# cmaestre/pcl_tracking

Measured on AMD Instinct MI355X. Metric: particles x input-points / sec per frame (tracked frames/sec @8192 particles per GPU), higher is better.
Workload: dtype f32

## Files before the change

include/pft.h:

```cpp
#ifndef PFT_H
#define PFT_H

#include <stddef.h>
#include <stdint.h>

#ifdef __cplusplus
extern "C" {
#endif

#define PFT_ABI_VERSION 5

typedef struct pft_point_xyzrgba {
  float x, y, z, w;
  uint32_t rgba;
  uint32_t pad[3];
} pft_point_xyzrgba;

typedef struct pft_particle {
  float x, y, z, w;
  float roll, pitch, yaw, weight;
} pft_particle;

typedef enum pft_status {
  PFT_OK = 0,
// ... 93 lines not shown
int pft_dist_begin_frame(pft_tracker* t);
int pft_dist_phase_a(pft_tracker* t, int iteration);
int pft_dist_phase_b(pft_tracker* t);
int pft_dist_phase_c(pft_tracker* t);

int pft_set_particles(pft_tracker* t, const pft_particle* p, size_t n);
int pft_eval_weights(pft_tracker* t, const pft_particle* particles, size_t P, float* raw_w, int32_t* nn_idx,
                     float* nn_d2);
int pft_debug_get_bbox(pft_tracker* t, float bbox[6]);
int pft_debug_get_crop(pft_tracker* t, int32_t* idx, size_t cap, size_t* n);
int pft_debug_get_octree(pft_tracker* t, int32_t* depth, double min_xyz[3], double max_xyz[3], uint32_t* n_leaves,
                         uint32_t* n_nodes);
int pft_debug_get_point_keys(pft_tracker* t, uint32_t* keys3, size_t cap_points);
int pft_debug_get_scan_stats(pft_tracker* t, uint64_t* queries, uint64_t* scanned_points);
int pft_debug_set_limits(pft_tracker* t, uint32_t max_words, int sorted_npass);
int pft_debug_state_save(pft_tracker* t);
int pft_debug_state_restore(pft_tracker* t);
int pft_debug_inject_error(pft_tracker* t, uint32_t bits);
int pft_debug_get_host_stat(pft_tracker* t, uint32_t out4[4]);
int pft_debug_get_ticks(pft_tracker* t, uint64_t* ticks32);
int pft_debug_get_descent_stats(pft_tracker* t, uint64_t* dbg32);
int pft_debug_get_hard_steps(pft_tracker* t, uint64_t out5[5]);
int pft_debug_get_likelihood_layout(pft_tracker* t, uint32_t out4[4]);
int pft_debug_aabb_support_subset(const pft_point_xyzrgba* pts, size_t n, uint32_t* keep, size_t* n_keep);
#ifdef PFT_DIAG
void pft_debug_set_ablate(pft_tracker* t, int mask);
#endif
int pft_debug_likelihood_occupancy(void);
int pft_debug_normalize(pft_tracker* t, float* w_inout, size_t n, double* fit_ratio);
int pft_debug_alias(pft_tracker* t, const float* w, size_t n, int32_t* a, double* q);
int pft_debug_weighted_mean(pft_tracker* t, const pft_particle* p, size_t n, pft_particle* out);
int pft_debug_init_particles(pft_tracker* t, const pft_particle* rep, uint32_t id_offset, size_t n_local,
                             pft_particle* out);
int pft_debug_resample(pft_tracker* t, const pft_particle* old, size_t n_total, const int32_t* a, const double* q,
                       const pft_particle* rep, uint32_t epoch, uint32_t id_offset, size_t n_local,
                       pft_particle* out);
int pft_debug_pose_to_matrix(pft_tracker* t, const pft_particle* p, size_t n, float* m12);
int pft_debug_kld_resample(pft_tracker* t, const pft_particle* old, size_t n_old, const int32_t* a, const double* q,
                           const pft_particle* motion, uint32_t epoch, pft_particle* out, int32_t* bins6,
                           uint32_t* n_out, uint32_t* k_out);
double pft_kld_normal_quantile(double u);
double pft_kld_bound(int k, double delta, double epsilon);

enum {
  PFT_K_RESAMPLE = 0, PFT_K_AABB = 1, PFT_K_CROP = 2, PFT_K_OCTREE = 3, PFT_K_LIKELIHOOD = 4,
  PFT_K_POPULATION = 5, PFT_K_PACK = 6, PFT_K_COUNT = 7
// ... 11 lines not shown
```

pcl_tracking_amd/_lib.py:

```python
import ctypes as C
import os

_HERE = os.path.dirname(os.path.abspath(__file__))
LIB_PATH = os.environ.get("PFT_LIB_PATH") or os.path.join(_HERE, "_build", "libpft_hip.so")

PFT_ABI_VERSION = 5
PFT_SUM_TREE, PFT_SUM_PCL = 0, 1
PFT_CD_RING = 32
K_RESAMPLE, K_AABB, K_CROP, K_OCTREE, K_LIKELIHOOD, K_POPULATION, K_PACK, K_COUNT = range(8)

STATUS = {0: "ok", 1: "invalid argument", 2: "no input cloud", 3: "no reference cloud", 4: "no usable HIP device",
          5: "HIP error", 6: "capacity exceeded", 7: "invalid state"}


class PftError(RuntimeError):
    def __init__(self, status, detail=""):
        self.status = status
        super().__init__("pft status %d (%s) %s" % (status, STATUS.get(status, "?"), detail))


class Config(C.Structure):
    _fields_ = [
        ("abi_version", C.c_uint32), ("device_id", C.c_int32), ("stream", C.c_void_p),
        ("stream_is_external", C.c_int32),
# ... 79 lines not shown
    ("pft_to_state", None, [_vp, _vp]),
    ("pft_get_fit_ratio", C.c_int, [_vp, _P(_f64)]),
    ("pft_synchronize", C.c_int, [_vp]),
    ("pft_dist_bind", C.c_int, [_vp, _vp, _vp, _vp]),
    ("pft_dist_begin_frame", C.c_int, [_vp]),
    ("pft_dist_phase_a", C.c_int, [_vp, C.c_int]),
    ("pft_dist_phase_b", C.c_int, [_vp]),
    ("pft_dist_phase_c", C.c_int, [_vp]),
    ("pft_set_particles", C.c_int, [_vp, _vp, _sz]),
    ("pft_eval_weights", C.c_int, [_vp, _vp, _sz, _vp, _vp, _vp]),
    ("pft_debug_get_bbox", C.c_int, [_vp, _vp]),
    ("pft_debug_get_crop", C.c_int, [_vp, _vp, _sz, _P(_sz)]),
    ("pft_debug_get_octree", C.c_int, [_vp, _P(_i32), _vp, _vp, _P(_u32), _P(_u32)]),
    ("pft_debug_get_point_keys", C.c_int, [_vp, _vp, _sz]),
    ("pft_debug_get_scan_stats", C.c_int, [_vp, _P(_u64), _P(_u64)]),
    ("pft_debug_set_limits", C.c_int, [_vp, _u32, C.c_int]),
    ("pft_debug_inject_error", C.c_int, [_vp, _u32]),
    ("pft_debug_state_save", C.c_int, [_vp]),
    ("pft_debug_state_restore", C.c_int, [_vp]),
    ("pft_debug_get_host_stat", C.c_int, [_vp, _vp]),
    ("pft_debug_get_ticks", C.c_int, [_vp, _vp]),
    ("pft_debug_get_descent_stats", C.c_int, [_vp, _vp]),
    ("pft_debug_get_likelihood_layout", C.c_int, [_vp, _vp]),
    ("pft_debug_get_hard_steps", C.c_int, [_vp, _vp]),
    ("pft_debug_aabb_support_subset", C.c_int, [_vp, C.c_size_t, _vp, _vp]),
    ("pft_debug_likelihood_occupancy", C.c_int, []),
    ("pft_debug_normalize", C.c_int, [_vp, _vp, _sz, _P(_f64)]),
    ("pft_debug_alias", C.c_int, [_vp, _vp, _sz, _vp, _vp]),
    ("pft_debug_weighted_mean", C.c_int, [_vp, _vp, _sz, _vp]),
    ("pft_debug_init_particles", C.c_int, [_vp, _vp, _u32, _sz, _vp]),
    ("pft_debug_resample", C.c_int, [_vp, _vp, _sz, _vp, _vp, _vp, _u32, _u32, _sz, _vp]),
    ("pft_debug_pose_to_matrix", C.c_int, [_vp, _vp, _sz, _vp]),
    ("pft_debug_kld_resample", C.c_int, [_vp, _vp, _sz, _vp, _vp, _vp, _u32, _vp, _vp, _P(_u32), _P(_u32)]),
    ("pft_set_change_detector", C.c_int, [_vp, C.c_int, C.c_int, C.c_int, _f64]),
    ("pft_get_change_detector", C.c_int, [_vp, _P(C.c_int), _P(C.c_int), _P(C.c_int), _P(_f64)]),
    ("pft_debug_change_state", C.c_int, [_vp, C.c_int, _P(_u32), _P(_u32), _vp, _P(_i32), _vp, _P(_u32)]),
    ("pft_debug_change_detect", C.c_int, [_vp, _vp, _sz, C.c_int, _f64, C.c_int, _vp, _sz, _P(_sz)]),
    ("pft_set_report_cloud", C.c_int, [_vp, _vp, _sz]),
    ("pft_report", C.c_int, [_vp]),
    ("pft_get_report", C.c_int, [_vp, _P(ObjectReport)]),
    ("pft_get_tracked_cloud", C.c_int, [_vp, _vp, _sz, _P(_sz)]),
    ("pft_kld_normal_quantile", _f64, [_f64]),
    ("pft_kld_bound", _f64, [C.c_int, _f64, _f64]),
    ("pft_profile_enable", C.c_int, [_vp, C.c_int]),
    ("pft_profile_get", C.c_int, [_vp, C.c_int, _P(_f64), _P(_u64)]),
    ("pft_profile_reset", C.c_int, [_vp]),
# ... 77 lines not shown
```

pcl_tracking_amd/csrc/pft_api.hip:

```cpp
#include <math.h>
#include <stdio.h>
#include <string.h>

#include <stdlib.h>

#include <algorithm>
#include <cmath>
#include <string>
#include <vector>

#include "pft_internal.h"

#define HIPCHK(t, call)                                                                       \
  do {                                                                                        \
    hipError_t e_ = (call);                                                                   \
    if (e_ != hipSuccess) {                                                                   \
      (t)->err = std::string(#call) + ": " + hipGetErrorString(e_);                           \
      return PFT_ERR_HIP;                                                                     \
    }                                                                                         \
  } while (0)

struct EvPair {
  hipEvent_t a, b;
};
// ... 13 lines not shown
  std::string err;

  pft_point_xyzrgba* d_ref_raw = nullptr;
  float4 *d_ref_xyz = nullptr, *d_ref_hsv = nullptr, *d_ref_box = nullptr;
  size_t bbox_part_cap = 0;
  uint32_t ref_cap = 0;
  pft_point_xyzrgba* d_in_raw = nullptr;
  float4* d_in_pts = nullptr;
  uint32_t in_cap = 0, N = 0;
  const pft_point_xyzrgba* raw_pending = nullptr;
  pft_particle* d_part[2] = {nullptr, nullptr};
  int cur = 0;
  float* d_mats = nullptr;
  float* d_bbox_part = nullptr;
  float* d_bbox6 = nullptr;
  uint32_t* d_crop_counts = nullptr;
  unsigned long long* d_crop_slots = nullptr;
  uint32_t crop_epoch = 0;
  float4* d_crop_pts = nullptr;
  int32_t* d_crop_idx = nullptr;
  uint32_t* d_words = nullptr;
  uint32_t max_words = 0;
  uint16_t* d_jump = nullptr;
  uint32_t* d_ref_perm = nullptr;
  float4* d_leaf_pts = nullptr;
  uint32_t *d_leaf_order = nullptr, *d_pt_node = nullptr, *d_pt_key = nullptr, *d_pt_tmp = nullptr;
  unsigned long long* d_pt_key64 = nullptr;
  SortBufs sort = {};
  uint32_t* h_stat = nullptr;
  PftSwitches sw = {};
  bool leaf_indirect = false;
  int force_npass = 0;
  uint32_t inject_error = 0;
  double* d_partial = nullptr;
  int32_t* d_alias_list = nullptr;
  double* d_alias_pref = nullptr;
  double* d_pop_part = nullptr;
  uint32_t *d_eg_start = nullptr, *d_eg_cnt = nullptr, *d_eg_tile = nullptr;
  uint32_t *d_ec_slot = nullptr, *d_ec_cells = nullptr, *d_ec_count = nullptr, *d_ec_base = nullptr;
  float4* d_ec_list = nullptr;
  uint32_t ec_pool_cap = 0;
  uint32_t *d_eq_cellq = nullptr, *d_eq_nq = nullptr, *d_eq_qbase = nullptr, *d_eq_bbase = nullptr, *d_eq_fill = nullptr,
           *d_eq_blk = nullptr, *d_eq_tiles = nullptr;
  float4* d_eq_sorted = nullptr;
  double* d_eq_out = nullptr;
  uint32_t eq_cap = 0, eq_blk_cap = 0, eq_tiles_cap = 0;
// ... 241 lines not shown
}

static void sync_dev(pft_tracker* t) {
  PftDev& d = t->dev;
  d.ref_xyz = t->d_ref_xyz;
  d.ref_box = t->d_ref_box;
  d.ref_hsv = t->d_ref_hsv;
  d.in_pts = t->d_in_pts;
  d.N = t->N;
  d.part_cur = t->d_part[t->cur];
  d.part_all = t->bound_gathered ? static_cast<pft_particle*>(t->bound_gathered) : t->d_part[t->cur];
  d.mats = t->d_mats;
  d.bbox_part = t->d_bbox_part;
  d.bbox_grid = (uint32_t)t->num_cus;
  d.bbox_part_cap = (uint32_t)t->bbox_part_cap;
  d.bbox6 = t->bound_bbox6 ? static_cast<float*>(t->bound_bbox6) : t->d_bbox6;
  d.crop_counts = t->d_crop_counts;
  d.crop_slots = t->d_crop_slots;
  d.crop_pts = t->d_crop_pts;
  d.crop_idx = t->d_crop_idx;
  d.words = t->d_words;
  d.max_words = t->max_words;
  d.jump = t->d_jump;
  d.ref_perm = t->d_ref_perm;
  d.leaf_pts = t->d_leaf_pts;
  d.leaf_order = t->d_leaf_order;
  d.pt_node = t->d_pt_node;
  d.pt_key = t->d_pt_key;
  d.pt_tmp = t->d_pt_tmp;
  d.pt_key64 = t->d_pt_key64;
  d.host_stat = t->h_stat;
  d.partial = t->d_partial;
  d.alias_list = t->d_alias_list;
  d.alias_pref = t->d_alias_pref;
  d.pop_part = t->d_pop_part;
  d.p_active = t->prm.kld ? &t->d_hdr->p_active : nullptr;
  d.eg_start = t->d_eg_start;
  d.eg_cnt = t->d_eg_cnt;
  d.eg_tile = t->d_eg_tile;
  d.eg_cap = t->d_eg_start ? PFT_EG_CAP : 0u;
  d.ec_slot = t->d_ec_slot;
  d.ec_cells = t->d_ec_cells;
  d.ec_count = t->d_ec_count;
  d.ec_base = t->d_ec_base;
  d.ec_list = t->d_ec_list;
  d.ec_pool_cap = t->ec_pool_cap;
// ... 119 lines not shown
      HIPCHK(t, hipMemcpyAsync(n.b.set_cnt[k], c.b.set_cnt[k], (size_t)c.b.cap * 4u, hipMemcpyDeviceToDevice, t->stream));
    }
    HIPCHK(t, hipStreamSynchronize(t->stream));
  } else {
    HIPCHK(t, hipMemsetAsync(n.b.st, 0, sizeof(PftChangeState), t->stream));
  }
  cd_free(c);
  c = n;
  return PFT_OK;
}

PftSwitches pft_read_switches() {
  auto on = [](const char* name) { return getenv(name) != nullptr; };
  auto is1 = [](const char* name) { const char* e = getenv(name); return e && e[0] == '1'; };
  PftSwitches w = {};
  w.graph = is1("PFT_GRAPH");
  if (const char* b = getenv("PFT_FORCE_BUILDER")) w.builder = !strcmp(b, "single") ? 1 : (!strcmp(b, "sorted") ? 2 : 0);
  w.leaf_indirect = on("PFT_LEAF_INDIRECT") ? (int)is1("PFT_LEAF_INDIRECT") : -1;
  w.aabb_full = on("PFT_AABB_FULL");
  w.resample_one_lane = on("PFT_RESAMPLE_ONE_LANE");
  w.split_resample = on("PFT_SPLIT_RESAMPLE") || w.resample_one_lane;
  w.crop_two_pass = on("PFT_CROP_TWO_PASS");
  w.generic_descent = is1("PFT_GENERIC_DESCENT");
  w.exact_path = on("PFT_EXACT_SHELLS_ONLY") ? PftExactPath::shells : on("PFT_EXACT_PER_QUERY") ? PftExactPath::per_query : PftExactPath::sorted;
#ifdef PFT_DIAG
  if (const char* a = getenv("PFT_ABLATE")) w.ablate = atoi(a);
  w.skip_octree = on("PFT_DEBUG_SKIP_OCTREE");
#endif
  return w;
}

#ifdef PFT_DIAG
extern "C" void pft_debug_set_ablate(pft_tracker* t, int mask) { if (t) t->sw.ablate = mask; }
#endif

extern "C" int pft_create(const pft_config* cfg, pft_tracker** out) {
  if (!cfg || !out) return PFT_ERR_INVALID_ARG;
  *out = nullptr;
  if (cfg->abi_version != PFT_ABI_VERSION || cfg->particle_num <= 0 || cfg->iteration_num <= 0 ||
      cfg->world_size <= 0 || cfg->rank < 0 || cfg->rank >= cfg->world_size || cfg->use_normal != 0 ||
      cfg->particle_num % cfg->world_size != 0 || !(cfg->octree_resolution > 0) ||
      (cfg->sum_order != PFT_SUM_TREE && cfg->sum_order != PFT_SUM_PCL))
    return PFT_ERR_INVALID_ARG;
  if (cfg->particle_num > PFT_MAX_PARTICLES) return PFT_ERR_CAPACITY;
  if (cfg->kld_adaptive) {
    if (cfg->world_size != 1 || cfg->maximum_particle_num <= 0 || !(cfg->kld_epsilon > 0)) return PFT_ERR_INVALID_ARG;
// ... 47 lines not shown
  p.M = 0;
  p.nchunk = 1;
  p.ref_chunk = PFT_REF_CHUNK;
  p.split_last = 0;
  p.kld = cfg->kld_adaptive ? 1u : 0u;
  p.kld_max = (uint32_t)cfg->maximum_particle_num;
  p.kld_z = pft_kld_normal_quantile(cfg->kld_delta);
  p.kld_eps = cfg->kld_epsilon;
  for (int k = 0; k < 6; k++) p.kld_bin[k] = (float)cfg->kld_bin_size[k];
  p.motion_ratio = cfg->motion_ratio;
  p.sum_order = cfg->sum_order;
  t->Pcap = p.kld && p.kld_max > p.P_total ? p.kld_max : p.P_total;

  const size_t Pl = p.kld ? t->Pcap : p.P_local, Pt = t->Pcap;
  hipError_t e = hipSuccess;
  auto A = [&](hipError_t r) { if (e == hipSuccess) e = r; };
  A(dalloc(&t->d_part[0], Pt));
  A(dalloc(&t->d_part[1], Pt));
  A(dalloc(&t->d_mats, Pl * 12));
  t->bbox_part_cap = std::max<size_t>((size_t)t->num_cus, (Pl * 4u + 255u) / 256u);
  A(dalloc(&t->d_bbox_part, t->bbox_part_cap * 6));
  A(dalloc(&t->d_bbox6, 8));
  A(dalloc(&t->d_jump, (size_t)1 << (3 * PFT_JUMP_MAX_LEVEL)));
  A(dalloc(&t->d_alias_list, 2 * Pt));
  A(dalloc(&t->d_alias_pref, 2 * Pt));
  A(dalloc(&t->d_pop_part, (size_t)PFT_POPM_MAX_WGS * 16));
  A(dalloc(&t->d_alias_pos, Pt));
  A(dalloc(&t->d_raw_w, Pt));
  if (cfg->exact_nearest) {
    A(dalloc(&t->d_eg_start, (size_t)PFT_EG_CAP + 1));
    A(dalloc(&t->d_eg_cnt, (size_t)PFT_EG_CAP));
    A(dalloc(&t->d_eg_tile, (size_t)PFT_EG_CAP / 2048 + 2));
    A(dalloc(&t->d_ec_slot, (size_t)PFT_EG_CAP));
    A(dalloc(&t->d_ec_cells, (size_t)PFT_EC_SLOTS));
    A(dalloc(&t->d_ec_count, (size_t)PFT_EC_SLOTS));
    A(dalloc(&t->d_ec_base, (size_t)PFT_EC_SLOTS));
    t->ec_pool_cap = PFT_EC_POOL_MIN;
    A(dalloc(&t->d_ec_list, (size_t)t->ec_pool_cap));
    A(dalloc(&t->d_eq_cellq, (size_t)PFT_EG_CAP));
    A(dalloc(&t->d_eq_nq, (size_t)PFT_EC_SLOTS));
    A(dalloc(&t->d_eq_qbase, (size_t)PFT_EC_SLOTS));
    A(dalloc(&t->d_eq_bbase, (size_t)PFT_EC_SLOTS));
    A(dalloc(&t->d_eq_fill, (size_t)PFT_EC_SLOTS));
  }
  if (p.kld) {
    A(dalloc(&t->d_kld_table, (size_t)6 * p.kld_max + 128));
// ... 17 lines not shown
    }
  }
  sync_dev(t);
  *out = t;
  return PFT_OK;
}

extern "C" void pft_destroy(pft_tracker* t) {
  if (!t) return;
  if (t->stream) hipStreamSynchronize(t->stream);
  if (t->graph_exec) hipGraphExecDestroy(t->graph_exec);
  for (int k = 0; k < PFT_K_COUNT; k++)
    for (auto& p : t->ev[k]) {
      hipEventDestroy(p.a);
      hipEventDestroy(p.b);
    }
  for (auto& p : t->ev_free) {
    hipEventDestroy(p.a);
    hipEventDestroy(p.b);
  }
  dfree(t->d_ref_raw); dfree(t->d_ref_xyz); dfree(t->d_ref_hsv); dfree(t->d_ref_box);
  dfree(t->d_in_raw); dfree(t->d_in_pts);
  dfree(t->d_part[0]); dfree(t->d_part[1]); dfree(t->d_mats); dfree(t->d_bbox_part); dfree(t->d_bbox6);
  dfree(t->d_crop_counts); dfree(t->d_crop_slots); dfree(t->d_crop_pts); dfree(t->d_crop_idx); dfree(t->d_words); dfree(t->d_jump); dfree(t->d_ref_perm);
  dfree(t->d_leaf_pts); dfree(t->d_leaf_order); dfree(t->d_pt_node); dfree(t->d_pt_key); dfree(t->d_pt_tmp);
  dfree(t->d_pt_key64); dfree(t->sort.keys[0]); dfree(t->sort.keys[1]); dfree(t->sort.vals[0]); dfree(t->sort.vals[1]);
  dfree(t->sort.hist); dfree(t->sort.tile_cnt); dfree(t->sort.tile_box); if (t->h_stat) hipHostFree(t->h_stat);
  dfree(t->d_partial); dfree(t->d_alias_list); dfree(t->d_alias_pos); dfree(t->d_raw_w);
  dfree(t->d_alias_pref); dfree(t->d_pop_part); dfree(t->d_kld_table); dfree(t->d_kld_bins); dfree(t->d_eg_start); dfree(t->d_eg_cnt); dfree(t->d_eg_tile); dfree(t->d_ec_slot); dfree(t->d_ec_cells); dfree(t->d_ec_count); dfree(t->d_ec_base); dfree(t->d_ec_list); dfree(t->d_eq_cellq); dfree(t->d_eq_nq); dfree(t->d_eq_qbase); dfree(t->d_eq_bbase); dfree(t->d_eq_fill); dfree(t->d_eq_blk); dfree(t->d_eq_tiles); dfree(t->d_eq_sorted); dfree(t->d_eq_out); dfree(t->d_hdr); dfree(t->d_nn_idx); dfree(t->d_nn_d2); dfree(t->d_dbg_part);
  dfree(t->d_dbg_hdr); dfree(t->d_dbg_f);
  dfree(t->sv_part); dfree(t->sv_alias_list); dfree(t->sv_alias_pref); dfree(t->sv_alias_pos); dfree(t->sv_hdr);
  cd_free(t->cd); cd_free(t->cd_dbg);
  dfree(t->d_rep_pts); dfree(t->d_rep_tracked); dfree(t->d_report);
  dfree(t->sv_cd); dfree(t->sv_cd_key[0]); dfree(t->sv_cd_key[1]); dfree(t->sv_cd_cnt[0]); dfree(t->sv_cd_cnt[1]);
  if (t->own_stream && t->stream) hipStreamDestroy(t->stream);
  delete t;
}

extern "C" const char* pft_last_error_string(const pft_tracker* t) { return t ? t->err.c_str() : "null handle"; }

extern "C" int pft_synchronize(pft_tracker* t) {
  if (!t) return PFT_ERR_INVALID_ARG;
  HIPCHK(t, hipStreamSynchronize(t->stream));
  return check_device_error(t);
}

extern "C" int pft_set_reference(pft_tracker* t, const pft_point_xyzrgba* pts, size_t n) {
// ... 271 lines not shown
    if (!keep_point_keys) db.pt_key = nullptr;
    const volatile uint32_t* hs = t->h_stat;
    const uint32_t last_n = hs ? hs[0] : 0u, last_depth = hs ? hs[1] : 0u;
    bool sorted = last_n > PFT_SORTED_BUILD_MIN;
    if (t->sw.builder == 1) sorted = false;
    if (t->sw.builder == 2) sorted = true;
#ifdef PFT_DIAG
    if (t->sw.skip_octree && ++t->dbg_builds > 8) {
    } else
#endif
    if (sorted) {
      int npass = last_depth > 0u ? (int)((3u * (last_depth + 1u) + 7u) / 8u) : 8;
      if (t->force_npass > 0) npass = t->force_npass;
      if (npass > 8) npass = 8;
      pftk_octree_sorted(t->stream, t->prm, db, t->sort, d.N, npass);
      t->leaf_indirect = false;
    } else {
      t->leaf_indirect = t->sw.leaf_indirect >= 0 ? t->sw.leaf_indirect == 1 : (unsigned long long)np * t->prm.M <= 8000000ull;
      pftk_octree(t->stream, t->prm, db, last_n, t->leaf_indirect);
    }
  }
  {
    ProfScope ps(t, PFT_K_LIKELIHOOD);
    const int flags = (t->sw.generic_descent ? 0 : 1) | (t->sw.ablate << 8);
    pftk_likelihood(t->stream, t->prm, d, np, debug_nn, t->num_cus, t->leaf_indirect, flags);
  }
}

static int check_ready(pft_tracker* t) {
  if (!t) return PFT_ERR_INVALID_ARG;
  hipSetDevice(t->cfg.device_id);
  if (!t->has_input || t->N == 0) return PFT_ERR_NO_INPUT;
  if (!t->has_ref) return PFT_ERR_NO_REFERENCE;
  return PFT_OK;
}

extern "C" int pft_compute(pft_tracker* t) {
  int r = check_ready(t);
  if (r != PFT_OK) return r;
  if (t->cfg.world_size != 1) {
    t->err = "pft_compute on a sharded handle: drive the pft_dist_* phases instead";
    return PFT_ERR_STATE;
  }
  if (!t->initialized) stage_init_particles(t);
  if (!t->cd_latched) {
    t->cd_res_latched = t->cd_res;
    t->cd_latched = true;
// ... 455 lines not shown
  PftHeader h;
  int r = read_hdr(t, &h);
  if (r != PFT_OK) return r;
  for (int i = 0; i < 32; i++) dbg32[i] = h.dbg[i];
  dbg32[30] = t->prm.M_box;
  dbg32[31] = t->prm.M;
  if (t->cfg.exact_nearest) {
    dbg32[8] = h.ec_nslots;
    dbg32[9] = h.ec_pool_used;
    dbg32[10] = h.eq_totals & 0xffffffffull;
    dbg32[11] = h.eq_totals >> 32;
    dbg32[12] = h.eg_ncells;
    dbg32[13] = h.n_crop;
  }
  return PFT_OK;
}

extern "C" int pft_debug_get_likelihood_layout(pft_tracker* t, uint32_t out4[4]) {
  if (!t || !out4) return PFT_ERR_INVALID_ARG;
  PftHeader h;
  int r = read_hdr(t, &h);
  if (r != PFT_OK) return r;
  memcpy(out4, h.lik_layout, sizeof(h.lik_layout));
  return PFT_OK;
}

extern "C" int pft_debug_get_hard_steps(pft_tracker* t, uint64_t out5[5]) {
  if (!t || !out5) return PFT_ERR_INVALID_ARG;
  PftHeader h;
  int r = read_hdr(t, &h);
  if (r != PFT_OK) return r;
  for (int i = 0; i < 5; i++) out5[i] = h.dbg_hard[i];
  return PFT_OK;
}

extern "C" int pft_debug_get_scan_stats(pft_tracker* t, uint64_t* queries, uint64_t* scanned) {
  if (!t) return PFT_ERR_INVALID_ARG;
  PftHeader h;
  int r = read_hdr(t, &h);
  if (r != PFT_OK) return r;
  if (queries) *queries = h.stat_queries;
  if (scanned) *scanned = h.stat_scanned;
  return PFT_OK;
}

struct DbgPop {
// ... 368 lines not shown
```

pcl_tracking_amd/csrc/pft_device_utils.h:

```cpp
#pragma once
#include <float.h>
#include <math.h>

#include "pft_internal.h"

#define WAVE 64
#define UNROLL_FENCE(j, every) do { if (((j) % (every)) == (every) - 1) __builtin_amdgcn_sched_barrier(0); } while (0)

__device__ __forceinline__ bool pft_unchanged(const uint32_t* gate) { return gate && *gate == 0u; }

__device__ __forceinline__ int lane_id() { return threadIdx.x & (WAVE - 1); }
__device__ __forceinline__ int wave_id() { return threadIdx.x >> 6; }

template <typename T>
__device__ __forceinline__ T wave_sum(T v) {
#pragma unroll
  for (int o = 32; o > 0; o >>= 1) v += __shfl_xor(v, o);
  return v;
}
template <int CTRL, int ROW_MASK>
__device__ __forceinline__ double dpp_move_f64(double v) {
  const unsigned long long b = (unsigned long long)__double_as_longlong(v);
  const int lo = __builtin_amdgcn_update_dpp(0, (int)(uint32_t)b, CTRL, ROW_MASK, 0xf, false);
  const int hi = __builtin_amdgcn_update_dpp(0, (int)(uint32_t)(b >> 32), CTRL, ROW_MASK, 0xf, false);
// ... 255 lines not shown
  *alias_if_large = (int32_t)k;
  const uint32_t pp = v.pos[k];
  if (!(pp >> 31) || v.m == 0) return q0;
  const uint32_t pos = pp & 0x7fffffffu;
  const double Ek = v.E[pos];
  const uint32_t is = upper_bound_gt2(v.D, v.m, Ek, v.cD, v.sD);
  if (is < v.m) {
    if (pos + 1 < v.nh) *alias_if_large = v.H[pos + 1];
    return 1.0 + Ek - v.D[is];
  }
  const double eprev = pos > 0 ? v.E[pos - 1] : -1.0;
  const double Dm = v.D[v.m - 1];
  if (Dm > eprev) return 1.0 + Ek - Dm;
  return q0;
}

__device__ __forceinline__ int32_t alias_a_small(const AliasView& v, uint32_t k) {
  if (v.nh == 0) return (int32_t)k;
  const uint32_t pos = v.pos[k] & 0x7fffffffu;
  const double dprev = pos > 0 ? v.D[pos - 1] : 0.0;
  const uint32_t kk = lower_bound_ge2(v.E, v.nh, dprev, v.cE, v.sE);
  return kk < v.nh ? v.H[kk] : (int32_t)k;
}
```

pcl_tracking_amd/csrc/pft_internal.h:

```cpp
#pragma once
#include <hip/hip_runtime.h>
#include <stdint.h>

#include <vector>

#include "../../include/pft.h"

#define PFT_MAX_DEVICES 64
#define PFT_MAX_DEPTH 30
#define PFT_TABLE_MAX_DEPTH 10
#define PFT_MAX_GROW 40
#define PFT_JUMP_MAX_LEVEL 4
#define PFT_REF_CHUNK 256
#ifndef PFT_BUILD_THREADS
#define PFT_BUILD_THREADS 1024
#endif
#ifndef PFT_LIK_GROUPS
#define PFT_LIK_GROUPS 64
#endif
#ifndef PFT_LIK_CTR_STRIDE
#define PFT_LIK_CTR_STRIDE 16u
#endif
#ifndef PFT_LIK_THREADS
#define PFT_LIK_THREADS 1024
#endif
#ifndef PFT_LIK_WGS_PER_CU
#define PFT_LIK_WGS_PER_CU 2
#endif
#define PFT_POP_THREADS 1024
#define PFT_SORTED_BUILD_MIN 18000
#define PFT_EG_CAP (1u << 21)
#define PFT_EC_SLOTS (1u << 19)
#define PFT_EC_POOL (1u << 24)
#define PFT_EC_POOL_MIN (1u << 20)
#define PFT_POPM_THREADS 256
// ... 23 lines not shown
  float kld_bin[6];
  double motion_ratio;
  int32_t sum_order;
};

struct PftHeader {
  float bbox[6];
  uint32_t n_crop;
  uint32_t error;
  double omin[3], omax[3];
  int32_t depth;
  int32_t use_table;
  uint32_t n_words;
  uint32_t n_leaves;
  uint32_t leaf_start;
  uint32_t lvl_start[PFT_MAX_DEPTH + 3];
  int32_t n_grow;
  int32_t build_path;
  int32_t leaf_indirect;
  int32_t jump_level;
  float margin_cells;
  float ominf[3];
  float inv_res;
  uint32_t grow_idx[PFT_MAX_GROW];
  uint32_t grow_shift[PFT_MAX_GROW];
  uint32_t grow_old_depth[PFT_MAX_GROW];
  double grow_min[PFT_MAX_GROW + 1][3];
  double fit_ratio;
  pft_particle rep;
  pft_particle motion;
  uint32_t alias_m, alias_nh;
  float eg_g, eg_inv_g, eg_min[3];
  int32_t eg_dim[3];
  uint32_t eg_ncells;
  uint32_t p_active;
  uint32_t kld_k;
  unsigned long long stat_queries, stat_scanned;
  unsigned long long dbg[32];
  unsigned long long ticks[32];
  alignas(128) uint32_t lik_ctr[PFT_LIK_GROUPS * PFT_LIK_CTR_STRIDE];
  alignas(128) uint32_t ec_nslots;
  uint32_t ec_pool_used;
  unsigned long long eq_totals;
  alignas(128) uint32_t crop_ticket;
  uint32_t pop_bar[4];
  unsigned long long dbg_hard[5];
  uint32_t lik_layout[4];
};

struct PftDev {
  const float4* ref_xyz;
  const float4* ref_hsv;
  const float4* ref_box;
  const float4* in_pts;
  uint32_t N;
  pft_particle* part_cur;
  pft_particle* part_all;
  float* mats;
  float* bbox_part;
  uint32_t bbox_grid;
  uint32_t bbox_part_cap;
  float* bbox6;
  uint32_t* crop_counts;
  unsigned long long* crop_slots;
  float4* crop_pts;
  int32_t* crop_idx;
  uint32_t* words;
  uint32_t max_words;
  uint16_t* jump;
  const uint32_t* ref_perm;
  float4* leaf_pts;
  uint32_t* leaf_order;
  uint32_t* pt_node;
  uint32_t* pt_key;
  unsigned long long* pt_key64;
  uint32_t* pt_tmp;
  double* partial;
  int32_t* alias_list;
  double* alias_pref;
  uint32_t* alias_pos;
  float* raw_w;
  double* pop_part;
  PftHeader* hdr;
  const uint32_t* p_active;
  uint32_t* eg_start;
  uint32_t* eg_cnt;
  uint32_t* eg_tile;
  uint32_t eg_cap;
  uint32_t* ec_slot;
  uint32_t* ec_cells;
  uint32_t* ec_count;
  uint32_t* ec_base;
// ... 37 lines not shown
  uint32_t* tab_cnt;
  unsigned long long* pt_key;
  uint32_t* mark;
  uint32_t cap, tab_cap;
};
struct PftChangeArgs {
  double res;
  uint32_t use, interval, min_points;
  uint32_t force;
};
void pftk_change_detect(hipStream_t s, const PftChangeBufs& b, const float4* pts, const uint32_t* n_ptr, uint32_t n,
                        const PftChangeArgs& a, uint32_t* host_stat);

enum class PftExactPath { sorted, per_query, shells };
struct PftSwitches {
  bool graph;
  int builder;
  int leaf_indirect;
  bool aabb_full;
  bool split_resample;
  bool resample_one_lane;
  bool crop_two_pass;
  bool generic_descent;
  PftExactPath exact_path;
  int ablate;
  bool skip_octree;
};
PftSwitches pft_read_switches();

void pftk_report(hipStream_t s, const pft_point_xyzrgba* pts, uint32_t n, const PftHeader* hdr, int sum_order,
                 pft_point_xyzrgba* tracked, pft_object_report* out);
void pftk_pack_reference(hipStream_t s, const pft_point_xyzrgba* d_pts, uint32_t n, int argorder, float4* xyz,
                         float4* hsv);
void pftk_pack_input(hipStream_t s, const pft_point_xyzrgba* d_pts, uint32_t n, float4* out);
void pftk_init_particles(hipStream_t s, const PftParams& p, pft_particle rep, pft_particle* out, float* mats,
                         PftHeader* hdr);
void pftk_resample(hipStream_t s, const PftParams& p, const PftDev& d, uint32_t epoch, pft_particle* out, bool one_lane);
void pftk_bbox_final(hipStream_t s, const PftDev& d);
uint32_t pftk_resample_box(hipStream_t s, const PftParams& p, const PftDev& d, uint32_t epoch, pft_particle* out);
void pftk_resample_table(hipStream_t s, const PftParams& p, const pft_particle* old, const int32_t* a,
                         const double* q, const PftHeader* hdr, uint32_t epoch, pft_particle* out);
void pftk_pose_to_matrix(hipStream_t s, const pft_particle* p, uint32_t n, float* mats);
void pftk_aabb(hipStream_t s, const PftParams& p, const PftDev& d, uint32_t n_particles, bool finalize);
void pft_aabb_support_subset(const pft_point_xyzrgba* pts, size_t n, std::vector<uint32_t>& keep);
void pftk_exact_grid(hipStream_t s, const PftParams& p, const PftDev& d);
void pftk_likelihood_exact(hipStream_t s, const PftParams& p, const PftDev& d, uint32_t n_particles, bool debug_nn,
// ... 28 lines not shown
```

pcl_tracking_amd/csrc/pft_likelihood.hip:

```cpp
#include "pft_device_utils.h"

#ifndef PFT_LIK_PENALTY
#define PFT_LIK_PENALTY 1
#endif

struct LikCtx {
  const uint32_t* words;
  const float* tab;
  uint32_t per_axis;
  const float* lut_h;
  const float* lut_s;
  const float* pen;
  const uint16_t* jump;
  int J;
  uint32_t lvlJ_start;
  float margin, near_thr, ominx, ominy, ominz, inv_res, ncell;
  uint32_t leaf0;
  const uint16_t* leaf16;
};

struct HybridWords {
  const __attribute__((address_space(3))) uint32_t* lds;
  const uint32_t* __restrict__ glob;
  uint32_t n_lds;
  __device__ __forceinline__ uint32_t operator[](uint32_t i) const { return i < n_lds ? lds[i] : glob[i]; }
};

__device__ __forceinline__ double rcp_nr(double x) {
  double r = __builtin_amdgcn_rcp(x);
  double e = fma(-x, r, 1.0);
  r = fma(r, e, r);
  e = fma(-x, r, 1.0);
  r = fma(r, e, r);
  return r;
}

__device__ __forceinline__ bool face_violation(uint32_t kx, uint32_t ky, uint32_t kz, uint32_t lowf, uint32_t highf,
                                               int sh) {
// ... 67 lines not shown
        }
        continue;
      }
      uint32_t node = 0, jx = 1, jy = 1, jz = 1;
      int lvl = 0;
      int dbg_fast = 0, dbg_gen = 0, dbg_jump = 0, dbg_hard = 0;
      if (FAST) {
        const float tx = (qx - cx.ominx) * cx.inv_res, ty = (qy - cx.ominy) * cx.inv_res,
                    tz = (qz - cx.ominz) * cx.inv_res;
        const float flx = floorf(tx), fly = floorf(ty), flz = floorf(tz);
        const bool inside = (int)(fminf(fminf(tx, ty), tz) >= 0.0f) & (int)(fmaxf(fmaxf(tx, ty), tz) < cx.ncell);
        const float fx = tx - flx, fy = ty - fly, fz = tz - flz;
        const float mg = cx.margin, mh = 1.0f - cx.margin;
        const uint32_t kx = inside ? (uint32_t)flx : 0u, ky = inside ? (uint32_t)fly : 0u,
                       kz = inside ? (uint32_t)flz : 0u;
        int V = -1;
        const float off = fmaxf(fmaxf(fabsf(fx - 0.5f), fabsf(fy - 0.5f)), fabsf(fz - 0.5f));
        if (__builtin_amdgcn_ballot_w64(off > cx.near_thr)) {
          const int vx = near_face_level(kx, fx < mg, fx > mh), vy = near_face_level(ky, fy < mg, fy > mh),
                    vz = near_face_level(kz, fz < mg, fz > mh);
          V = max(vx, max(vy, vz));
        }
        V = inside ? V : 31;
        const int lim = min(D, D - 1 - V);
        if (cx.J > 0) {
          const int sh = D - cx.J;
          const uint32_t e = cx.jump[(kx >> sh) | ((ky >> sh) << cx.J) | ((kz >> sh) << (2 * cx.J))];
          const bool take = (cx.J <= lim) & (e != 0u);
          node = take ? cx.lvlJ_start + e - 1u : 0u;
          lvl = take ? cx.J : 0;
          if (DEBUG_NN) dbg_jump = take ? 1 : 0;
        }
        while (lvl < lim) {
          const int sh = D - lvl - 1;
          const uint32_t c = (((kx >> sh) & 1u) << 2) | (((ky >> sh) & 1u) << 1) | ((kz >> sh) & 1u);
          const uint32_t wv = W[node];
          if (!((wv >> c) & 1u)) break;
          node = (wv >> 8) + __popc(wv & 0xffu & ((1u << c) - 1u));
          lvl++;
          dbg_fast++;
        }
        const int up = D - lvl;
        const uint32_t top = 1u << lvl;
        jx = (kx >> up) | top; jy = (ky >> up) | top; jz = (kz >> up) | top;
      }
      if ((abl & 1) && lvl < D) {
        node = cx.leaf0;
        lvl = D;
      }
      for (; lvl < D; lvl++) {
        dbg_gen++;
        const uint32_t wv = W[node];
        const uint32_t mask = wv & 0xffu, base = wv >> 8;
// ... 273 lines not shown
    uint32_t* dst = reinterpret_cast<uint32_t*>(ljump);
    for (uint32_t i = threadIdx.x; i < jump_bytes / 4u; i += blockDim.x) dst[i] = src[i];
  }
  if (words_in_lds || branch_only) {
    const uint32_t nb = leaf16 ? leaf_start : n_words;
    for (uint32_t i = threadIdx.x; i < nb; i += blockDim.x) lwords[i] = d.words[i];
    if (leaf16 && !branch_only)
      for (uint32_t i = threadIdx.x; i <= n_leaves; i += blockDim.x) lleaf[i] = (uint16_t)d.words[leaf_start + i];
  } else {
    for (uint32_t i = threadIdx.x; i < n_lds_words; i += blockDim.x) lwords[i] = d.words[i];
  }
  __syncthreads();

  LikCtx cx;
  cx.words = nullptr;
  cx.tab = tab;
  cx.per_axis = per_axis;
  cx.lut_h = lut_h;
  cx.lut_s = lut_s;
  cx.pen = pen;
  cx.jump = ljump;
  cx.J = J;
  cx.lvlJ_start = J > 0 ? hdr->lvl_start[J] : 0u;
  cx.margin = hdr->margin_cells;
  cx.near_thr = 0.5f - 1.01f * hdr->margin_cells - 1.0e-6f;
  cx.ominx = hdr->ominf[0];
  cx.ominy = hdr->ominf[1];
  cx.ominz = hdr->ominf[2];
  cx.inv_res = hdr->inv_res;
  cx.ncell = (float)(1u << (D > 0 ? D : 0));
  cx.leaf0 = hdr->leaf_start;
  cx.leaf16 = lleaf;
  if (branch_only) {
    const uint32_t* W = lwords;
    if (fast)
      PFT_LIK_RUN(true, true, 2);
    else
      PFT_LIK_RUN(true, false, 2);
  } else if (words_in_lds && leaf16) {
    const uint32_t* W = lwords;
    if (fast)
      PFT_LIK_RUN(true, true, 1);
    else if (use_tab)
      PFT_LIK_RUN(true, false, 1);
    else
      PFT_LIK_RUN(false, false, 1);
// ... 70 lines not shown
```

pcl_tracking_amd/csrc/pft_octree.hip:

```cpp
#include "pft_device_utils.h"

#ifdef PFT_DIAG
#define STAMP(k) do { if (threadIdx.x == 0) d.hdr->ticks[k] = wall_clock64(); } while (0)
#define TICK_NOW() wall_clock64()
#else
#define STAMP(k) do { } while (0)
#define TICK_NOW() 0ull
#endif

#include "pft_octree_box.h"

#define PFT_REPLAY_HEAD 1024u
__device__ __forceinline__ void box_replay(BuildSh& S, const float4* __restrict__ pts, uint32_t n, double res, unsigned long long* hdr_ticks) {
  const uint32_t tid = threadIdx.x, nt = blockDim.x;
  const uint32_t head = n < PFT_REPLAY_HEAD ? n : PFT_REPLAY_HEAD;
  float lmn[3] = {FLT_MAX, FLT_MAX, FLT_MAX}, lmx[3] = {-FLT_MAX, -FLT_MAX, -FLT_MAX};
  const uint32_t wt = tid - WAVE, ws = nt - WAVE;
  auto local_aabb = [&]() {
    for (uint32_t i0 = PFT_REPLAY_HEAD + wt; i0 < n; i0 += 8u * ws) {
      float4 q[8];
#pragma unroll
      for (uint32_t k = 0; k < 8u; k++) q[k] = pts[min(i0 + k * ws, n - 1u)];
#pragma unroll
      for (uint32_t k = 0; k < 8u; k++) {
// ... 522 lines not shown
  if (tid == 0) {
    hdr->error = S.err;
    hdr->depth = D;
    hdr->use_table = use_table;
    hdr->n_grow = S.ngrow;
    hdr->build_path = path;
    hdr->leaf_indirect = copy_leaf_pts == 2 ? 1 : 0;
    if (d.host_stat) d.host_stat[1] = (uint32_t)D;
    hdr->jump_level = (ok && use_table) ? S.jump : 0;
    hdr->n_leaves = ok ? n_leaves : 0;
    hdr->leaf_start = ok ? leaf_start : 0;
    hdr->n_words = ok ? leaf_start + n_leaves + 1 : 0;
  }
  if (tid == 64) {
    double maxabs = 0.0;
    for (int a = 0; a < 3; a++) maxabs = fmax(maxabs, fmax(fabs(S.mn[a]), fabs(S.mx[a])));
    const double eta = maxabs * 1.1920928955078125e-07;
    const double s_top = prm.res * (double)(1u << (D > 0 ? D - 1 : 0));
    const double E = 9.0 * eta + 40.0 * 5.9604644775390625e-08 * s_top;
    double mc = 2.0 * E / prm.res + 1.0e-3;
    hdr->margin_cells = (float)(mc < 0.25 ? mc : 1.0);
  }
  if (tid == 128) hdr->inv_res = (float)(1.0 / prm.res);
  if (tid >= 192 && tid < 195) {
    const int a = (int)tid - 192;
    hdr->ominf[a] = (float)S.mn[a];
    hdr->omin[a] = n > 0 ? S.mn[a] : 0.0;
    hdr->omax[a] = n > 0 ? S.mx[a] : 0.0;
  }
  if (tid >= 256 && tid < 256 + PFT_MAX_DEPTH + 3 && (int)tid - 256 <= D + 1) hdr->lvl_start[tid - 256] = S.lvl[tid - 256];
}

template <bool GATED>
__global__ __launch_bounds__(256) void k_leaf_gather(PftDev d) {
  if (GATED && pft_unchanged(d.gate)) return;
  const PftHeader* hdr = d.hdr;
  const uint32_t pos = blockIdx.x * 256u + threadIdx.x;
  if (hdr->error || hdr->depth <= 0 || pos >= hdr->n_crop) return;
  d.leaf_pts[pos] = d.crop_pts[d.leaf_order[pos]];
}

#ifndef PFT_OCTREE_GATED_TU
extern template __global__ void k_octree_build<true>(PftParams, PftDev, uint32_t, int, int);
extern template __global__ void k_leaf_gather<true>(PftDev);

static void pftk_octree_set_attr() {
  static bool attr_set[PFT_MAX_DEVICES];
  const uint32_t lds = ((uint32_t)pftk_max_lds_bytes() - 10240u) & ~15u;
  const int dev = pftk_cur_device();
  if (!attr_set[dev])
    attr_set[dev] = hipFuncSetAttribute(reinterpret_cast<const void*>(&k_octree_build<false>),
                                        hipFuncAttributeMaxDynamicSharedMemorySize, (int)lds) == hipSuccess &&
                    hipFuncSetAttribute(reinterpret_cast<const void*>(&k_octree_build<true>),
                                        hipFuncAttributeMaxDynamicSharedMemorySize, (int)lds) == hipSuccess;
}

void pftk_octree(hipStream_t s, const PftParams& p, const PftDev& d, uint32_t expected_points, bool indirect) {
  const uint32_t lds = ((uint32_t)pftk_max_lds_bytes() - 10240u) & ~15u;
  pftk_octree_set_attr();
  const int mode = indirect ? 2 : (expected_points <= 5000u ? 1 : 0);
  const dim3 gg((d.N + 255u) / 256u ? (d.N + 255u) / 256u : 1u);
  if (d.gate) {
// ... 18 lines not shown
```

pcl_tracking_amd/csrc/pft_octree_sorted.hip:

```cpp
#include "pft_device_utils.h"

#define SO_TILE 1024
#define SO_BINS 256

struct ReplaySh {
  double mn[3], mx[3];
  int depth, ngrow;
  uint32_t cur, err;
  uint32_t u32s[40];
};

__device__ void so_box_grow(ReplaySh& S, PftHeader* hdr, float4 p, uint32_t idx, double res) {
  const double epsd = (double)FLT_EPSILON;
  for (;;) {
    bool lx = p.x < S.mn[0], ly = p.y < S.mn[1], lz = p.z < S.mn[2];
    bool ux = p.x >= S.mx[0], uy = p.y >= S.mx[1], uz = p.z >= S.mx[2];
    if (!(lx || ly || lz || ux || uy || uz)) break;
    int g = S.ngrow;
    if (g >= PFT_MAX_GROW || S.depth >= PFT_MAX_DEPTH) {
      S.err |= 2u;
      break;
    }
    double side = (double)(1u << S.depth) * res;
    hdr->grow_idx[g] = idx;
// ... 131 lines not shown
    for (uint32_t j = tid; j < (1u << (3 * J - 1)); j += nt) jz[j] = 0u;
  }
  if (tid == 0) {
    hdr->error = S.err;
    hdr->depth = D;
    hdr->use_table = use_table;
    hdr->n_grow = S.ngrow;
    hdr->build_path = 2;
    hdr->leaf_indirect = 0;
    hdr->jump_level = (ok && use_table) ? J : 0;
    double maxabs = 0.0;
    for (int a = 0; a < 3; a++) maxabs = fmax(maxabs, fmax(fabs(S.mn[a]), fabs(S.mx[a])));
    const double eta = maxabs * 1.1920928955078125e-07;
    const double s_top = res * (double)(1u << (D > 0 ? D - 1 : 0));
    const double E = 9.0 * eta + 40.0 * 5.9604644775390625e-08 * s_top;
    double mc = 2.0 * E / res + 1.0e-3;
    hdr->margin_cells = (float)(mc < 0.25 ? mc : 1.0);
    for (int a = 0; a < 3; a++) {
      hdr->ominf[a] = (float)S.mn[a];
      hdr->omin[a] = n > 0 ? S.mn[a] : 0.0;
      hdr->omax[a] = n > 0 ? S.mx[a] : 0.0;
    }
    hdr->inv_res = (float)(1.0 / res);
    if (!ok) {
      hdr->n_words = 0;
      hdr->n_leaves = 0;
      hdr->leaf_start = 0;
    }
  }
}

__global__ void k_so_keys(PftParams prm, PftDev d, SortBufs sb, uint32_t n_pad) {
  if (pft_unchanged(d.gate)) return;
  const uint32_t i = blockIdx.x * blockDim.x + threadIdx.x;
  if (i >= n_pad) return;
  const PftHeader* hdr = d.hdr;
  const uint32_t n = hdr->n_crop;
  const int D = hdr->depth, ngrow = hdr->n_grow;
  if (i >= n || hdr->error || D <= 0) return;
  const double res = prm.res, inv_res = 1.0 / prm.res;
  const float4 p = d.crop_pts[i];
  int e = 0;
  while (e < ngrow && hdr->grow_idx[e] <= i) e++;
  const double tq[3] = {(double)p.x - hdr->grow_min[e][0], (double)p.y - hdr->grow_min[e][1],
                        (double)p.z - hdr->grow_min[e][2]};
  uint32_t kk[3];
// ... 301 lines not shown
```

Baseline: 804.9 billion.

## Add precomputed ancestor table to skip octree descent levels in likelihood

Adds a dense ancestor table that covers the crop bounding box at depth D minus two. During leaf gather, each table cell stores the deepest existing octree node reached for that coarse cell. The likelihood kernel then looks up this entry to start the descent near the leaves instead of walking from the jump level, and falls back to the jump table only when a wavefront has misses. This removes several dependent word loads per query, at the cost of extra table fill work, a buffer of up to 1 MiB, and epoch bookkeeping to keep the table consistent with the tree. It is enabled by default and only on the direct-leaf, table-built path.

```diff
diff --git a/include/pft.h b/include/pft.h
--- a/include/pft.h
+++ b/include/pft.h
@@ -139,6 +139,7 @@
 int pft_debug_get_descent_stats(pft_tracker* t, uint64_t* dbg32);
 int pft_debug_get_hard_steps(pft_tracker* t, uint64_t out5[5]);
 int pft_debug_get_likelihood_layout(pft_tracker* t, uint32_t out4[4]);
+int pft_debug_get_ancestor_table(pft_tracker* t, uint32_t info10[10], uint32_t* table, size_t cap);
 int pft_debug_aabb_support_subset(const pft_point_xyzrgba* pts, size_t n, uint32_t* keep, size_t* n_keep);
 #ifdef PFT_DIAG
 void pft_debug_set_ablate(pft_tracker* t, int mask);
diff --git a/pcl_tracking_amd/_lib.py b/pcl_tracking_amd/_lib.py
--- a/pcl_tracking_amd/_lib.py
+++ b/pcl_tracking_amd/_lib.py
@@ -125,6 +125,7 @@
     ("pft_debug_get_ticks", C.c_int, [_vp, _vp]),
     ("pft_debug_get_descent_stats", C.c_int, [_vp, _vp]),
     ("pft_debug_get_likelihood_layout", C.c_int, [_vp, _vp]),
+    ("pft_debug_get_ancestor_table", C.c_int, [_vp, _vp, _vp, _sz]),
     ("pft_debug_get_hard_steps", C.c_int, [_vp, _vp]),
     ("pft_debug_aabb_support_subset", C.c_int, [_vp, C.c_size_t, _vp, _vp]),
     ("pft_debug_likelihood_occupancy", C.c_int, []),
diff --git a/pcl_tracking_amd/csrc/pft_api.hip b/pcl_tracking_amd/csrc/pft_api.hip
--- a/pcl_tracking_amd/csrc/pft_api.hip
+++ b/pcl_tracking_amd/csrc/pft_api.hip
@@ -59,6 +59,7 @@
   uint32_t* d_words = nullptr;
   uint32_t max_words = 0;
   uint16_t* d_jump = nullptr;
+  uint32_t* d_anc = nullptr;
   uint32_t* d_ref_perm = nullptr;
   float4* d_leaf_pts = nullptr;
   uint32_t *d_leaf_order = nullptr, *d_pt_node = nullptr, *d_pt_key = nullptr, *d_pt_tmp = nullptr;
@@ -346,6 +347,7 @@
   d.words = t->d_words;
   d.max_words = t->max_words;
   d.jump = t->d_jump;
+  d.anc = t->d_anc;
   d.ref_perm = t->d_ref_perm;
   d.leaf_pts = t->d_leaf_pts;
   d.leaf_order = t->d_leaf_order;
@@ -511,6 +513,7 @@
   w.split_resample = on("PFT_SPLIT_RESAMPLE") || w.resample_one_lane;
   w.crop_two_pass = on("PFT_CROP_TWO_PASS");
   w.generic_descent = is1("PFT_GENERIC_DESCENT");
+  w.ancestor_table = !on("PFT_ANCESTOR_TABLE") || is1("PFT_ANCESTOR_TABLE");
   w.exact_path = on("PFT_EXACT_SHELLS_ONLY") ? PftExactPath::shells : on("PFT_EXACT_PER_QUERY") ? PftExactPath::per_query : PftExactPath::sorted;
 #ifdef PFT_DIAG
   if (const char* a = getenv("PFT_ABLATE")) w.ablate = atoi(a);
@@ -604,6 +607,7 @@
   A(dalloc(&t->d_bbox_part, t->bbox_part_cap * 6));
   A(dalloc(&t->d_bbox6, 8));
   A(dalloc(&t->d_jump, (size_t)1 << (3 * PFT_JUMP_MAX_LEVEL)));
+  if (t->sw.ancestor_table) A(dalloc(&t->d_anc, PFT_ANC_CAP));
   A(dalloc(&t->d_alias_list, 2 * Pt));
   A(dalloc(&t->d_alias_pref, 2 * Pt));
   A(dalloc(&t->d_pop_part, (size_t)PFT_POPM_MAX_WGS * 16));
@@ -667,7 +671,7 @@
   dfree(t->d_ref_raw); dfree(t->d_ref_xyz); dfree(t->d_ref_hsv); dfree(t->d_ref_box);
   dfree(t->d_in_raw); dfree(t->d_in_pts);
   dfree(t->d_part[0]); dfree(t->d_part[1]); dfree(t->d_mats); dfree(t->d_bbox_part); dfree(t->d_bbox6);
-  dfree(t->d_crop_counts); dfree(t->d_crop_slots); dfree(t->d_crop_pts); dfree(t->d_crop_idx); dfree(t->d_words); dfree(t->d_jump); dfree(t->d_ref_perm);
+  dfree(t->d_crop_counts); dfree(t->d_crop_slots); dfree(t->d_crop_pts); dfree(t->d_crop_idx); dfree(t->d_words); dfree(t->d_jump); dfree(t->d_anc); dfree(t->d_ref_perm);
   dfree(t->d_leaf_pts); dfree(t->d_leaf_order); dfree(t->d_pt_node); dfree(t->d_pt_key); dfree(t->d_pt_tmp);
   dfree(t->d_pt_key64); dfree(t->sort.keys[0]); dfree(t->sort.keys[1]); dfree(t->sort.vals[0]); dfree(t->sort.vals[1]);
   dfree(t->sort.hist); dfree(t->sort.tile_cnt); dfree(t->sort.tile_box); if (t->h_stat) hipHostFree(t->h_stat);
@@ -985,7 +989,7 @@
   }
   {
     ProfScope ps(t, PFT_K_LIKELIHOOD);
-    const int flags = (t->sw.generic_descent ? 0 : 1) | (t->sw.ablate << 8);
+    const int flags = (t->sw.generic_descent ? 0 : 1) | (t->sw.ancestor_table ? 2 : 0) | (t->sw.ablate << 8);
     pftk_likelihood(t->stream, t->prm, d, np, debug_nn, t->num_cus, t->leaf_indirect, flags);
   }
 }
@@ -1487,6 +1491,28 @@
   int r = read_hdr(t, &h);
   if (r != PFT_OK) return r;
   memcpy(out4, h.lik_layout, sizeof(h.lik_layout));
+  return PFT_OK;
+}
+
+extern "C" int pft_debug_get_ancestor_table(pft_tracker* t, uint32_t info10[10], uint32_t* table, size_t cap) {
+  if (!t || !info10) return PFT_ERR_INVALID_ARG;
+  PftHeader h;
+  int r = read_hdr(t, &h);
+  if (r != PFT_OK) return r;
+  const bool has = t->d_anc != nullptr && h.anc_level > 0;
+  info10[0] = has && h.anc_epoch == h.build_epoch ? 1u : 0u;
+  info10[1] = has ? (uint32_t)h.anc_level : 0u;
+  for (int a = 0; a < 3; a++) {
+    info10[2 + a] = has ? h.anc_lo[a] : 0u;
+    info10[5 + a] = has ? h.anc_bits[a] : 0u;
+  }
+  info10[8] = h.build_epoch;
+  info10[9] = h.anc_epoch;
+  const size_t cells = has ? (size_t)1 << (h.anc_bits[0] + h.anc_bits[1] + h.anc_bits[2]) : 0u;
+  if (table && cells && cap) {
+    HIPCHK(t, hipMemcpyAsync(table, t->d_anc, std::min(cap, cells) * sizeof(uint32_t), hipMemcpyDeviceToHost, t->stream));
+    HIPCHK(t, hipStreamSynchronize(t->stream));
+  }
   return PFT_OK;
 }
 
diff --git a/pcl_tracking_amd/csrc/pft_device_utils.h b/pcl_tracking_amd/csrc/pft_device_utils.h
--- a/pcl_tracking_amd/csrc/pft_device_utils.h
+++ b/pcl_tracking_amd/csrc/pft_device_utils.h
@@ -301,3 +301,29 @@
   const uint32_t kk = lower_bound_ge2(v.E, v.nh, dprev, v.cE, v.sE);
   return kk < v.nh ? v.H[kk] : (int32_t)k;
 }
+
+__device__ inline void pft_anc_window(PftHeader* hdr, const PftDev& d, int D, bool on, const double mn[3], double res) {
+  const int L = D - PFT_ANC_UP;
+  on = on && d.anc != nullptr && L >= 1;
+  const float inv = (float)(1.0 / res);
+  uint32_t lo[3] = {0u, 0u, 0u}, bits[3] = {0u, 0u, 0u};
+  for (int a = 0; a < 3 && on; a++) {
+    const float om = (float)mn[a];
+    const float f0 = fmaxf(floorf((hdr->bbox[2 * a] - om) * inv), 0.0f);
+    const float f1 = fmaxf(floorf((hdr->bbox[2 * a + 1] - om) * inv), 0.0f);
+    const uint32_t top = (1u << L) - 1u;
+    const uint32_t c0 = min(f0 < 2147483648.0f ? (uint32_t)f0 >> PFT_ANC_UP : top, top);
+    const uint32_t c1 = min(f1 < 2147483648.0f ? (uint32_t)f1 >> PFT_ANC_UP : top, top);
+    on = c1 >= c0;
+    const uint32_t n = c1 - c0 + 1u;
+    bits[a] = n > 1u ? 32u - (uint32_t)__clz((int)(n - 1u)) : 0u;
+    lo[a] = min(c0, (1u << L) - (1u << bits[a]));
+  }
+  on = on && bits[0] + bits[1] + bits[2] <= PFT_ANC_CAP_BITS;
+  hdr->anc_level = on ? L : 0;
+  for (int a = 0; a < 3; a++) {
+    hdr->anc_lo[a] = on ? lo[a] : 0u;
+    hdr->anc_bits[a] = on ? bits[a] : 0u;
+  }
+  hdr->build_epoch = hdr->build_epoch + 1u;
+}
diff --git a/pcl_tracking_amd/csrc/pft_internal.h b/pcl_tracking_amd/csrc/pft_internal.h
--- a/pcl_tracking_amd/csrc/pft_internal.h
+++ b/pcl_tracking_amd/csrc/pft_internal.h
@@ -11,6 +11,13 @@
 #define PFT_TABLE_MAX_DEPTH 10
 #define PFT_MAX_GROW 40
 #define PFT_JUMP_MAX_LEVEL 4
+#ifndef PFT_ANC_CAP_BITS
+#define PFT_ANC_CAP_BITS 18
+#endif
+#define PFT_ANC_CAP (1u << PFT_ANC_CAP_BITS)
+#ifndef PFT_ANC_UP
+#define PFT_ANC_UP 2
+#endif
 #define PFT_REF_CHUNK 256
 #ifndef PFT_BUILD_THREADS
 #define PFT_BUILD_THREADS 1024
@@ -80,6 +87,10 @@
   float margin_cells;
   float ominf[3];
   float inv_res;
+  int32_t anc_level;
+  uint32_t anc_lo[3], anc_bits[3];
+  uint32_t build_epoch;
+  uint32_t anc_epoch;
   uint32_t grow_idx[PFT_MAX_GROW];
   uint32_t grow_shift[PFT_MAX_GROW];
   uint32_t grow_old_depth[PFT_MAX_GROW];
@@ -126,6 +137,7 @@
   uint32_t* words;
   uint32_t max_words;
   uint16_t* jump;
+  uint32_t* anc;
   const uint32_t* ref_perm;
   float4* leaf_pts;
   uint32_t* leaf_order;
@@ -209,6 +221,7 @@
   bool resample_one_lane;
   bool crop_two_pass;
   bool generic_descent;
+  bool ancestor_table;
   PftExactPath exact_path;
   int ablate;
   bool skip_octree;
diff --git a/pcl_tracking_amd/csrc/pft_likelihood.hip b/pcl_tracking_amd/csrc/pft_likelihood.hip
--- a/pcl_tracking_amd/csrc/pft_likelihood.hip
+++ b/pcl_tracking_amd/csrc/pft_likelihood.hip
@@ -14,6 +14,8 @@
   const uint16_t* jump;
   int J;
   uint32_t lvlJ_start;
+  const uint32_t* anc;
+  uint32_t alo, abits;
   float margin, near_thr, ominx, ominy, ominz, inv_res, ncell;
   uint32_t leaf0;
   const uint16_t* leaf16;
@@ -127,13 +129,27 @@
           V = max(vx, max(vy, vz));
         }
         V = inside ? V : 31;
-        const int lim = min(D, D - 1 - V);
-        if (cx.J > 0) {
+        int lim = min(D, D - 1 - V);
+        bool inw = false;
+        uint32_t ae = 0u;
+        if (!INDIRECT && LEAF == 1 && cx.anc) {
+          const uint32_t bx = cx.abits & 0xffu, by = (cx.abits >> 8) & 0xffu, bz = cx.abits >> 16;
+          const uint32_t ux = (kx >> PFT_ANC_UP) - (cx.alo & 1023u), uy = (ky >> PFT_ANC_UP) - ((cx.alo >> 10) & 1023u),
+                         uz = (kz >> PFT_ANC_UP) - (cx.alo >> 20);
+          inw = ((ux >> bx) | (uy >> by) | (uz >> bz)) == 0u;
+          ae = cx.anc[inw ? ux | (uy << bx) | (uz << (bx + by)) : 0u];
+        }
+        const int a = (int)(ae >> 27);
+        const bool hit = inw & (a <= lim);
+        node = hit ? (ae & 0x7ffffffu) : 0u;
+        lvl = hit ? a : 0;
+        lim = (hit & (a < D - PFT_ANC_UP)) ? a : lim;
+        if (cx.J > 0 && __builtin_amdgcn_ballot_w64(!hit)) {
           const int sh = D - cx.J;
           const uint32_t e = cx.jump[(kx >> sh) | ((ky >> sh) << cx.J) | ((kz >> sh) << (2 * cx.J))];
-          const bool take = (cx.J <= lim) & (e != 0u);
-          node = take ? cx.lvlJ_start + e - 1u : 0u;
-          lvl = take ? cx.J : 0;
+          const bool take = !hit & (cx.J <= lim) & (e != 0u);
+          node = take ? cx.lvlJ_start + e - 1u : node;
+          lvl = take ? cx.J : lvl;
           if (DEBUG_NN) dbg_jump = take ? 1 : 0;
         }
         while (lvl < lim) {
@@ -453,6 +469,11 @@
   cx.jump = ljump;
   cx.J = J;
   cx.lvlJ_start = J > 0 ? hdr->lvl_start[J] : 0u;
+  const bool anc_on = fast && (flags & 2) && d.anc && hdr->anc_level > 0 && hdr->anc_epoch == hdr->build_epoch;
+  cx.anc = anc_on ? d.anc : nullptr;
+  static_assert(PFT_TABLE_MAX_DEPTH <= 10, "ancestor table window coordinates are packed in 10 bits");
+  cx.alo = hdr->anc_lo[0] | (hdr->anc_lo[1] << 10) | (hdr->anc_lo[2] << 20);
+  cx.abits = hdr->anc_bits[0] | (hdr->anc_bits[1] << 8) | (hdr->anc_bits[2] << 16);
   cx.margin = hdr->margin_cells;
   cx.near_thr = 0.5f - 1.01f * hdr->margin_cells - 1.0e-6f;
   cx.ominx = hdr->ominf[0];
diff --git a/pcl_tracking_amd/csrc/pft_octree.hip b/pcl_tracking_amd/csrc/pft_octree.hip
--- a/pcl_tracking_amd/csrc/pft_octree.hip
+++ b/pcl_tracking_amd/csrc/pft_octree.hip
@@ -568,6 +568,7 @@
     hdr->margin_cells = (float)(mc < 0.25 ? mc : 1.0);
   }
   if (tid == 128) hdr->inv_res = (float)(1.0 / prm.res);
+  if (tid == 320) pft_anc_window(hdr, d, D, ok && use_table && copy_leaf_pts == 0, S.mn, prm.res);
   if (tid >= 192 && tid < 195) {
     const int a = (int)tid - 192;
     hdr->ominf[a] = (float)S.mn[a];
@@ -577,13 +578,44 @@
   if (tid >= 256 && tid < 256 + PFT_MAX_DEPTH + 3 && (int)tid - 256 <= D + 1) hdr->lvl_start[tid - 256] = S.lvl[tid - 256];
 }
 
+__device__ __forceinline__ void anc_fill(const PftDev& d, uint32_t gid, uint32_t stride) {
+  const PftHeader* hdr = d.hdr;
+  const int L = hdr->anc_level;
+  if (L <= 0) return;
+  const uint32_t bx = hdr->anc_bits[0], by = hdr->anc_bits[1], n = 1u << (bx + by + hdr->anc_bits[2]);
+  const uint32_t x0 = hdr->anc_lo[0], y0 = hdr->anc_lo[1], z0 = hdr->anc_lo[2];
+  const int J = hdr->jump_level <= L ? hdr->jump_level : 0;
+  const uint32_t lvlJ = J > 0 ? hdr->lvl_start[J] : 0u;
+  for (uint32_t c = gid; c < n; c += stride) {
+    const uint32_t x = x0 + (c & ((1u << bx) - 1u)), y = y0 + ((c >> bx) & ((1u << by) - 1u)), z = z0 + (c >> (bx + by));
+    uint32_t node = 0;
+    int lvl = 0;
+    if (J > 0) {
+      const int sh = L - J;
+      const uint32_t e = d.jump[(x >> sh) | ((y >> sh) << J) | ((z >> sh) << (2 * J))];
+      node = e ? lvlJ + e - 1u : 0u;
+      lvl = e ? J : 0;
+    }
+    for (; lvl < L; lvl++) {
+      const int sh = L - lvl - 1;
+      const uint32_t ch = (((x >> sh) & 1u) << 2) | (((y >> sh) & 1u) << 1) | ((z >> sh) & 1u);
+      const uint32_t wv = d.words[node];
+      if (!((wv >> ch) & 1u)) break;
+      node = (wv >> 8) + __popc(wv & 0xffu & ((1u << ch) - 1u));
+    }
+    d.anc[c] = ((uint32_t)lvl << 27) | node;
+  }
+  if (gid == 0) d.hdr->anc_epoch = hdr->build_epoch;
+}
+
 template <bool GATED>
 __global__ __launch_bounds__(256) void k_leaf_gather(PftDev d) {
   if (GATED && pft_unchanged(d.gate)) return;
   const PftHeader* hdr = d.hdr;
   const uint32_t pos = blockIdx.x * 256u + threadIdx.x;
-  if (hdr->error || hdr->depth <= 0 || pos >= hdr->n_crop) return;
-  d.leaf_pts[pos] = d.crop_pts[d.leaf_order[pos]];
+  if (hdr->error || hdr->depth <= 0) return;
+  if (pos < hdr->n_crop) d.leaf_pts[pos] = d.crop_pts[d.leaf_order[pos]];
+  anc_fill(d, pos, gridDim.x * 256u);
 }
 
 #ifndef PFT_OCTREE_GATED_TU
diff --git a/pcl_tracking_amd/csrc/pft_octree_sorted.hip b/pcl_tracking_amd/csrc/pft_octree_sorted.hip
--- a/pcl_tracking_amd/csrc/pft_octree_sorted.hip
+++ b/pcl_tracking_amd/csrc/pft_octree_sorted.hip
@@ -177,6 +177,7 @@
       hdr->omax[a] = n > 0 ? S.mx[a] : 0.0;
     }
     hdr->inv_res = (float)(1.0 / res);
+    pft_anc_window(hdr, d, D, false, S.mn, res);
     if (!ok) {
       hdr->n_words = 0;
       hdr->n_leaves = 0;
```

Result: faster. 834.2 billion (median of 6 runs) (+3.6%).
